# yhao-wang/DenseRetrievalToolkits

Hardware: AMD Instinct MI355X
Metric: queries/sec@top-1000, 10Mx768 corpus (BASELINE: passages encoded/sec + queries/sec@top-1000, 10Mx768 corpus, 1/2/4/8 GPU) (higher is better)
Workload: dtype bf16

## Files before the change

### denseretrievaltoolkits_amd/_native.py

```python
from __future__ import annotations

import ctypes
import os
import threading

import torch

from .build_native import LIB_PATH

DRT_OK = 0
DRT_EINVAL = -1
ROW_STATS_LEN = 34

_lock = threading.Lock()
_lib = None

c_i32 = ctypes.c_int32
c_i64 = ctypes.c_int64
c_sz = ctypes.c_size_t
c_vp = ctypes.c_void_p
c_f32 = ctypes.c_float
c_u64 = ctypes.c_uint64

_SIGNATURES = [
    ("drt_version", ctypes.c_char_p, []),
    ("drt_ip_topk_workspace", c_sz, [c_i64, c_i64, c_i32, c_i32]),
    ("drt_ip_topk_bf16", c_i32, [c_vp, c_i64, c_vp, c_i64, c_i32, c_i32, c_i64, c_vp, c_vp, c_vp, c_vp, c_sz, c_vp]),
    ("drt_ip_topk_resolve_workspace", c_sz, [c_i64, c_i64, c_i32]),
    ("drt_ip_topk_resolve", c_i32, [c_vp, c_i64, c_vp, c_i64, c_i32, c_i32, c_i64, c_vp, c_vp, c_vp, c_vp, c_sz,
                                    c_vp, c_vp]),
    ("drt_topk_merge", c_i32, [c_vp, c_vp, c_i64, c_i32, c_i32, c_i32, c_vp, c_vp, c_vp]),
    ("drt_ip_topk_sample_rank", c_i32, [c_i32]),
    ("drt_ip_topk_dist_workspace", c_sz, [c_i64, c_i64, c_i64, c_i32, c_i32]),
    ("drt_ip_topk_dist_sample", c_i32, [c_vp, c_i64, c_vp, c_i64, c_i64, c_i32, c_i32, c_vp, c_vp, c_sz, c_vp]),
    ("drt_ip_topk_dist_tau", c_i32, [c_vp, c_i64, c_i32, c_i32, c_vp, c_vp]),
    ("drt_ip_topk_dist_filter", c_i32, [c_vp, c_i64, c_vp, c_i64, c_i64, c_i32, c_i32, c_i64, c_vp, c_vp, c_vp,
                                        c_sz, c_vp]),
    ("drt_ip_topk_dist_filter_chunks", c_i32, [c_vp, c_i64, c_vp, c_i64, c_i64, c_i32, c_i32, c_i64, c_vp, c_vp,
                                               c_vp, c_i32, c_vp, c_sz, c_vp]),
    ("drt_ip_topk_tighten_rank", c_i32, [c_i64, c_i32, c_i32]),
    ("drt_ip_topk_filter_passes_workspace", c_sz, [c_i64, c_i64, c_i64, c_i32, c_i32]),
    ("drt_ip_topk_filter_passes", c_i32, [c_vp, c_i64, c_vp, c_i64, c_i64, c_i32, c_i32, c_i64, c_vp, c_vp,
                                          c_i32, c_i32, c_vp, c_vp, c_vp, c_sz, c_vp]),
    ("drt_ip_topk_dist_filter_lists", c_i32, [c_vp, c_i64, c_vp, c_i64, c_i64, c_i32, c_i32, c_i64, c_vp, c_i32,
                                              c_vp, c_vp, c_vp, c_sz, c_vp]),
    ("drt_ip_topk_dist_filter_lists_at", c_i32, [c_vp, c_i64, c_vp, c_i64, c_i64, c_i32, c_i32, c_i64, c_vp,
                                                 c_i32, c_i64, c_vp, c_vp, c_vp, c_sz, c_vp]),
    ("drt_topk_merge_packed", c_i32, [c_vp, c_i64, c_i32, c_i32, c_i64, c_vp, c_vp, c_vp, c_vp]),
    ("drt_topk_merge_packed_cert", c_i32, [c_vp, c_i64, c_i32, c_i32, c_i32, c_i64, c_vp, c_vp, c_vp, c_vp]),
    ("drt_topk_merge_packed_capped", c_i32, [c_vp, c_i64, c_i32, c_i32, c_i32, c_i32, c_i64, c_vp, c_vp, c_vp,
                                             c_vp]),
    ("drt_row_stats_bf16", c_i32, [c_vp, c_i64, c_i32, c_vp, c_i32, c_vp]),
    ("drt_refine_width", c_i32, [c_i32]),
    ("drt_ip_topk_exact_bf16", c_i32, [c_vp, c_i64, c_vp, c_i64, c_i32, c_i32, c_i64, c_vp, c_vp, c_vp, c_vp, c_vp,
                                       c_sz, c_vp]),
    ("drt_hit_metrics_i8", c_i32, [c_vp, c_i64, c_i64, c_vp, c_i32, c_vp, c_vp]),
    ("drt_answer_match_i32", c_i32, [c_vp, c_i32, c_vp, c_vp, c_i64, c_i64, c_i64, c_vp, c_vp, c_i32, c_i32, c_vp,
# ... 98 lines not shown
PROF_SCAN, PROF_SAMPLE, PROF_SELECT, PROF_MERGE, PROF_GEMM = range(5)

EXPORTED = [n for n, _, _ in _SIGNATURES]


def lib_path() -> str:
    return os.environ.get("DRT_LIB", LIB_PATH)


def load():
    global _lib
    if _lib is not None:
        return _lib
    with _lock:
        if _lib is not None:
            return _lib
        path = lib_path()
        if not os.path.exists(path):
            raise RuntimeError(
                f"DRT native library not found at {path}; build it with "
                "`python -m denseretrievaltoolkits_amd.build_native` (no CPU fallback exists)")
        lib = ctypes.CDLL(path, mode=ctypes.RTLD_LOCAL)
        for name, res, args in _SIGNATURES:
            fn = getattr(lib, name)
            fn.restype = res
            fn.argtypes = args
        _lib = lib
    return _lib


def check(rc: int, what: str) -> None:
    if rc != DRT_OK:
        if rc == DRT_EINVAL:
            raise ValueError(f"{what}: invalid argument (DRT_EINVAL)")
        raise RuntimeError(f"{what}: HIP error {rc}")


def stream_ptr(device=None) -> int:
    return torch.cuda.current_stream(device).cuda_stream
```

### denseretrievaltoolkits_amd/csrc/search.hip

```cpp
#include <cmath>

#include "profile.h"
#include "search_internal.h"

namespace drt {

constexpr int kHitCap = 1024;
constexpr int kTopRL = 4;

__host__ __device__ __forceinline__ int pass_tiles(int ntiles, int npass, int pass) {
  return npass <= 1 ? ntiles : (pass < ntiles ? (ntiles - 1 - pass) / npass + 1 : 0);
}

__device__ __forceinline__ void glds16(const void* gsrc, uint32_t lds_addr) {
  uint32_t keep;
  asm volatile(
      "s_mov_b32 %0, m0\n\t"
      "s_mov_b32 m0, %2\n\t"
      "s_nop 0\n\t"
      "global_load_lds_dwordx4 %1, off\n\t"
      "s_mov_b32 m0, %0"
      : "=&s"(keep)
      : "v"(gsrc), "s"(lds_addr)
      : "memory");
// ... 108 lines not shown
  using C = Scan16Cfg<D, NW>;
  const int rsub = lane >> 3, pos = lane & 7;
#pragma unroll
  for (int j = 0; j < C::GLDS_PER_WAVE; ++j) {
    int J = j * NW + wave;
    if (C::GLDS_PER_TILE % NW != 0) J %= C::GLDS_PER_TILE;
    const int g = J >> 1;
    const int row = ((J & 1) << 3) + rsub;
    int64_t li = tile * kT16 + row;
    li = li < a.nrows ? li : a.nrows - 1;
    const int c = pos ^ ((row >> 1) & 7);
    const __bf16* src = a.P + (a.row0 + li * a.rstride) * a.ldp + g * 64 + c * 8;
    if (NTL) glds16_nt(src, __builtin_amdgcn_readfirstlane(buf_lds + J * 1024));
    else glds16(src, __builtin_amdgcn_readfirstlane(buf_lds + J * 1024));
  }
}

template <int D, int NW>
struct LeanTile {
  using C = Scan16Cfg<D, NW>;
  static constexpr int G = C::GLDS_PER_WAVE;
  uint32_t voff[G];
  uint32_t loff[G];
  __device__ __forceinline__ void init(const ScanArgs& a, int wave, int lane) {
    const int rsub = lane >> 3, pos = lane & 7;
#pragma unroll
    for (int j = 0; j < G; ++j) {
      int J = j * NW + wave;
      if (C::GLDS_PER_TILE % NW != 0) J %= C::GLDS_PER_TILE;
      const int g = J >> 1;
      const int row = ((J & 1) << 3) + rsub;
      const int c = pos ^ ((row >> 1) & 7);
      voff[j] = (uint32_t)((row * a.ldp + g * 64 + c * 8) * 2);
      loff[j] = (uint32_t)__builtin_amdgcn_readfirstlane(J * 1024);
    }
  }
  template <bool NT>
  __device__ __forceinline__ void issue(const ScanArgs& a, uint32_t slot_lds, const char* base, bool partial,
                                        int64_t tile, int wave, int lane) {
    if (partial) {
      issue_tile16<D, NW, NT>(a, slot_lds, tile, wave, lane);
      return;
    }
#define DRT_LEAN3(POL)                                                                                   \
  {                                                                                                     \
    uint32_t keep;                                                                                      \
    asm volatile(                                                                                       \
        "s_mov_b32 %0, m0\n\t"                                                                          \
        "s_mov_b32 m0, %2\n\t"                                                                          \
        "s_nop 0\n\t"                                                                                   \
        "global_load_lds_dwordx4 %3, %1" POL "\n\t"                                                     \
        "s_mov_b32 m0, %4\n\t"                                                                          \
        "s_nop 0\n\t"                                                                                   \
        "global_load_lds_dwordx4 %5, %1" POL "\n\t"                                                     \
        "s_mov_b32 m0, %6\n\t"                                                                          \
        "s_nop 0\n\t"                                                                                   \
// ... 19 lines not shown
  }
    if constexpr (G == 3) {
      if constexpr (NT) DRT_LEAN3(" nt")
      else DRT_LEAN3("")
    } else {
#pragma unroll
      for (int j = 0; j < G; ++j) {
        if constexpr (NT) DRT_LEAN1(" nt", j)
        else DRT_LEAN1("", j)
      }
    }
#undef DRT_LEAN3
#undef DRT_LEAN1
  }
};

template <int D>
struct HalfTile {
  using C = Scan16Cfg<D, 4>;
  static constexpr bool kOk = C::GLDS_PER_TILE % 4 == 0 && C::GLDS_PER_TILE <= 24;
  static constexpr int G = C::GLDS_PER_TILE / 4;
  uint32_t voff;
  uint32_t loff;
  __device__ __forceinline__ void init(const ScanArgs& a, int wave, int lane) {
    const int lw = wave & 3;
    const int row = ((lw & 1) << 3) + (lane >> 3);
    const int c = (lane & 7) ^ ((row >> 1) & 7);
    voff = (uint32_t)((row * a.ldp + (lw >> 1) * 64 + c * 8) * 2);
    loff = (uint32_t)__builtin_amdgcn_readfirstlane(lw * 1024);
  }
  __device__ __forceinline__ void issue(const ScanArgs& a, uint32_t slot_lds, const char* base, bool partial,
                                        int tile, int wave, int lane) {
    static_assert(kOk, "loader half: a multiple of four pieces per tile");
    uint32_t v = voff;
    if (partial) {
      const int row = ((wave & 1) << 3) + (lane >> 3);
      const int last = (int)(a.nrows - 1 - (int64_t)tile * kT16);
      if (row > last) v -= (uint32_t)((row - last) * a.ldp * 2);
    }
    const uint32_t l0 = slot_lds + loff;
    uint32_t keep;
#define DRT_HALF_PIECE(LDS, OFF) \
  "s_add_u32 m0, %2, " #LDS "\n\ts_nop 0\n\tglobal_load_lds_dwordx4 %3, %1 offset:" #OFF "\n\t"
#define DRT_HALF_ISSUE(PIECES) \
  asm volatile("s_mov_b32 %0, m0\n\t" PIECES "s_mov_b32 m0, %0" : "=&s"(keep) : "s"(base), "s"(l0), "v"(v) : "memory", "scc")
#define DRT_HP0 DRT_HALF_PIECE(0, 0)
#define DRT_HP1 DRT_HP0 DRT_HALF_PIECE(3840, 256)
#define DRT_HP2 DRT_HP1 DRT_HALF_PIECE(7680, 512)
#define DRT_HP3 DRT_HP2 DRT_HALF_PIECE(11520, 768)
#define DRT_HP4 DRT_HP3 DRT_HALF_PIECE(15360, 1024)
#define DRT_HP5 DRT_HP4 DRT_HALF_PIECE(19200, 1280)
    if constexpr (G == 1) DRT_HALF_ISSUE(DRT_HP0);
    else if constexpr (G == 2) DRT_HALF_ISSUE(DRT_HP1);
    else if constexpr (G == 3) DRT_HALF_ISSUE(DRT_HP2);
    else if constexpr (G == 4) DRT_HALF_ISSUE(DRT_HP3);
    else if constexpr (G == 5) DRT_HALF_ISSUE(DRT_HP4);
    else DRT_HALF_ISSUE(DRT_HP5);
#undef DRT_HP5
#undef DRT_HP4
#undef DRT_HP3
#undef DRT_HP2
// ... 420 lines not shown
  }
  if (my_tiles & 1) epilogue(accA, rbA);
  else epilogue(accB, rbB);
  if (wcnt) wave_flush_hits(a, qw, hk, hq, wcnt, lane);
}

template <int D>
struct Scan32Cfg {
  static constexpr int KS = D / 32;
  static constexpr int RD = KS % 2 == 0 ? 2 : 1;
  static constexpr int TILE_BYTES = kT16 * D * 2;
  static constexpr int HIT_BYTES = kHitCap * 9;
  static constexpr int NB_RAW = (160 * 1024 - HIT_BYTES) / TILE_BYTES;
  static constexpr int NB = NB_RAW > 6 ? 6 : NB_RAW;
  static constexpr int RING_BYTES = NB * TILE_BYTES;
  static constexpr int LDS_BYTES = RING_BYTES + HIT_BYTES;
  static_assert(NB >= 3, "ring too small");
  static_assert(LDS_BYTES <= 160 * 1024, "LDS budget");
};
constexpr int kQueriesPerWG32 = 256;

template <int D>
__global__ __launch_bounds__(512, 1) void ip_scan32r_kernel(ScanArgs a) {
  constexpr int NW = 8;
  using C = Scan16Cfg<D, NW>;
  using C32 = Scan32Cfg<D>;
  constexpr int NB = C32::NB;
  constexpr int PD = NB - 2;
  static_assert(NB == 6, "the pair protocol's slot census");
  constexpr int KS = C32::KS;
  constexpr int RD = C32::RD;
  constexpr int kSeg = kHitCap / NW;
  __shared__ __attribute__((aligned(16))) char smem[C32::LDS_BYTES];

  const int tid = threadIdx.x;
  const int wave = __builtin_amdgcn_readfirstlane(tid >> 6);
  const int lane = tid & 63;
  const int r = lane & 15;
  const int kq = lane >> 4;
  uint64_t* hk = (uint64_t*)(smem + C32::RING_BYTES) + wave * kSeg;
  uint8_t* hq = (uint8_t*)(smem + C32::RING_BYTES + kHitCap * 8) + wave * kSeg;

  const int64_t qbase = (int64_t)blockIdx.y * kQueriesPerWG32;
  const int tmul = a.npass > 1 ? a.npass : 1;
  const int tph = a.npass > 1 ? a.pass : 0;
  const int tall = (int)((a.nrows + kT16 - 1) / kT16);
  const int ntiles = pass_tiles(tall, a.npass, a.pass);
  const uint32_t nrows = (uint32_t)a.nrows;
  const int t0 = blockIdx.x;
  const int tstep = gridDim.x;
  const int my_tiles = t0 < ntiles ? (ntiles - 1 - t0) / tstep + 1 : 0;
  if (my_tiles == 0) return;
  const int partial_tile = ((a.nrows & (kT16 - 1)) != 0 && (tall - 1) % tmul == tph) ? ntiles - 1 : -1;
  const uint32_t ring = lds_addr_of(smem);
  constexpr bool HALVES = HalfTile<D>::kOk;
  constexpr int GW = HALVES ? HalfTile<D>::G : C::GLDS_PER_WAVE;
  constexpr int KDMA = HALVES ? KS / 12 : KS / 4;
  const bool loader = !HALVES || wave >= NW / 2;
  const int64_t tile_stride = (int64_t)tstep * tmul * kT16 * a.ldp * 2;
  const char* next_base = (const char*)(a.P + ((int64_t)t0 * tmul + tph) * kT16 * a.ldp);

  const int64_t qw = qbase + wave * 32;
  bf16x8 qf0[KS], qf1[KS];
  float tau0, tau1;
  {
    const int64_t g0 = qw + r, g1 = qw + 16 + r;
    const bool ok0 = g0 < a.nq, ok1 = g1 < a.nq;
    const int64_t s0 = ok0 ? g0 : 0, s1 = ok1 ? g1 : 0;
#pragma unroll
    for (int s = 0; s < KS; ++s) {
      qf0[s] = *(const bf16x8*)(a.Q + s0 * a.ldq + s * 32 + kq * 8);
      qf1[s] = *(const bf16x8*)(a.Q + s1 * a.ldq + s * 32 + kq * 8);
    }
    const float v0 = a.tau[s0], v1 = a.tau[s1];
    tau0 = ok0 ? v0 : __builtin_nanf("");
    tau1 = ok1 ? v1 : __builtin_nanf("");
    if (!ok0) {
#pragma unroll
      for (int s = 0; s < KS; ++s) qf0[s] = (bf16x8){};
    }
    if (!ok1) {
#pragma unroll
      for (int s = 0; s < KS; ++s) qf1[s] = (bf16x8){};
    }
  }
#pragma unroll
  for (int s = 0; s < KS; ++s) asm volatile("" ::"v"(qf0[s]), "v"(qf1[s]));
  asm volatile("" ::"v"(tau0), "v"(tau1));
  asm volatile("s_waitcnt vmcnt(0)" ::: "memory");

  LeanTile<D, NW> lt;
  HalfTile<D> ht;
  if constexpr (HALVES) ht.init(a, wave, lane);
  else lt.init(a, wave, lane);
  auto issue = [&](int slot, int tile) {
    if constexpr (HALVES)
      ht.issue(a, ring + slot * C::TILE_BYTES, next_base, tile == partial_tile, tile * tmul + tph, wave, lane);
    else
      lt.template issue<false>(a, ring + slot * C::TILE_BYTES, next_base, tile == partial_tile, tile * tmul + tph,
                               wave, lane);
    next_base += tile_stride;
  };
  auto pair_wait = [&](int it) {
    if (loader && it + PD <= my_tiles) wait_vmcnt<GW>();
    else wait_vmcnt<0>();
  };
#pragma unroll
  for (int p = 0; p < PD; ++p) {
    if (p < my_tiles && loader) issue(p, t0 + p * tstep);
  }
  if (wave >= NW / 2) __builtin_amdgcn_s_setprio(1);
  pair_wait(0);
  lds_barrier();

  const int sw = (r >> 1) & 7;
  int aoff[2];
#pragma unroll
  for (int m = 0; m < 2; ++m) aoff[m] = r * 128 + (((4 * m + kq) ^ sw) << 4);
  auto frag = [&](int slot, int s) -> bf16x8 {
    return *(const bf16x8*)(smem + slot * C::TILE_BYTES + (s >> 1) * (kT16 * 128) + aoff[s & 1]);
  };
  bf16x8 af[RD];
#pragma unroll
  for (int s = 0; s < RD; ++s) af[s] = frag(0, s);

  int wcnt = 0;
  auto append = [&](const f32x4& acc, float tau, int ql, uint32_t rowbase) {
    const float mx = fmaxf(fmaxf(acc[0], acc[1]), fmaxf(acc[2], acc[3])) - tau;
    if (__ballot(mx >= 0.0f) == 0ull) return;
#pragma unroll
    for (int j = 0; j < 4; ++j) {
      const bool hit = acc[j] >= tau && rowbase + j < nrows;
      const uint64_t m = __ballot(hit);
      if (m == 0ull) continue;
      const int c = __builtin_popcountll(m);
      if (wcnt + c > kSeg) {
        wave_flush_hits(a, qw, hk, hq, wcnt, lane);
        wcnt = 0;
      }
      if (hit) {
        const int pos = wcnt + (int)__builtin_amdgcn_mbcnt_hi((uint32_t)(m >> 32),
                                                              __builtin_amdgcn_mbcnt_lo((uint32_t)m, 0u));
        hk[pos] = ((uint64_t)desc_key(acc[j]) << 32) | (uint64_t)(a.row_base + rowbase + j);
        hq[pos] = (uint8_t)ql;
      }
      wcnt += c;
    }
  };

  auto epilogue = [&](const f32x4& p0, const f32x4& p1, uint32_t rowbase) {
    append(p0, tau0, r, rowbase);
    append(p1, tau1, 16 + r, rowbase);
  };

  int buf = 0;
  auto pair_sync = [&](int it) {
    pair_wait(it);
    lds_barrier();
  };
  auto iter = [&](int it, f32x4& acc0, f32x4& acc1, uint32_t& rb, const f32x4& prev0, const f32x4& prev1,
                  uint32_t rb_prev) {
    const int tile = t0 + it * tstep;
    const bool do_dma = it + PD < my_tiles && loader;
    const int ntile = tile + PD * tstep;
    const int pslot = buf < 2 ? buf + NB - 2 : buf - 2;
    const int nslot = buf + 1 == NB ? 0 : buf + 1;
    acc0 = (f32x4){0.f, 0.f, 0.f, 0.f};
    acc1 = (f32x4){0.f, 0.f, 0.f, 0.f};
#pragma unroll
    for (int s = 0; s < KS; ++s) {
      acc0 = __builtin_amdgcn_mfma_f32_16x16x32_bf16(af[s % RD], qf0[s], acc0, 0, 0, 0);
      acc1 = __builtin_amdgcn_mfma_f32_16x16x32_bf16(af[s % RD], qf1[s], acc1, 0, 0, 0);
      af[s % RD] = s + RD < KS ? frag(buf, s + RD) : frag(nslot, s + RD - KS);
      __builtin_amdgcn_sched_barrier(0);
      if (s == KDMA && do_dma) issue(pslot, ntile);
      __builtin_amdgcn_sched_barrier(0);
    }
    if (it > 0) epilogue(prev0, prev1, rb_prev);
    rb = (uint32_t)(tile * tmul + tph) * kT16 + 4 * kq;
    buf = nslot;
  };
  f32x4 a0, a1, b0, b1;
  uint32_t rbA = 0, rbB = 0;
  for (int it = 0; it < my_tiles; it += 2) {
    if (it > 0) pair_sync(it);
    iter(it, a0, a1, rbA, b0, b1, rbB);
    if (it + 1 < my_tiles) iter(it + 1, b0, b1, rbB, a0, a1, rbA);
  }
  if (my_tiles & 1) epilogue(a0, a1, rbA);
  else epilogue(b0, b1, rbB);
  if (wcnt) wave_flush_hits(a, qw, hk, hq, wcnt, lane);
}

struct TopkPlan : PlanHead {
  int64_t n, k, nq, nq_pad;
  bool sample;
  int64_t cap;
  int64_t m;
  int64_t stride;
  int64_t r;
  int64_t nchunk;
  int64_t kc;
  size_t off_cs, off_ci, off_delta, off_rcnt, total;
};

static size_t plan_refine_tail(TopkPlan& p) {
  p.kc = refine_width(p.k);
  WsBump b{p.head_end};
  p.off_cs = b.take((size_t)p.nq_pad * p.kc * 4);
  p.off_ci = b.take((size_t)p.nq_pad * p.kc * 8);
  p.off_delta = b.take((size_t)p.nq_pad * p.kc * 4);
  p.off_rcnt = b.take((size_t)p.nq_pad * 8);
  return b.o;
}
// ... 86 lines not shown
static int scan_grid_x(int64_t ntiles) {
  int dev = 0, cus = 256;
  if (hipGetDevice(&dev) == hipSuccess) {
    int v = 0;
    if (hipDeviceGetAttribute(&v, hipDeviceAttributeMultiprocessorCount, dev) == hipSuccess && v > 0)
      cus = v;
  }
  const int64_t g = std::min<int64_t>(ntiles, (int64_t)cus);
  return (int)std::max<int64_t>(g, 1);
}

static dim3 scan16_grid(int64_t nq, int64_t nrows, int qpw = kQueriesPerWG) {
  const unsigned gy = (unsigned)((nq + qpw - 1) / qpw);
  const int64_t ntiles = (nrows + kT16 - 1) / kT16;
  int gx = scan_grid_x(ntiles);
  if (gy > 1 && ntiles >= 8) {
    const int cus = scan_grid_x((int64_t)1 << 40);
    const int share = std::max(8, (cus / (int)gy) & ~7);
    gx = (int)std::min<int64_t>(ntiles, share);
  }
  return dim3(gx, gy);
}

template <int D>
static int launch_scan_d(const ScanArgs& a, int mode, hipStream_t s) {
  if (a.nq == 0 || a.nrows == 0) return DRT_OK;
  constexpr bool kLean = D <= 768;
  if (a.npass > 1 && (mode != SCAN_FILTER || !kLean || a.row0 != 0 || a.rstride != 1 || a.pass < 0 ||
                      a.pass >= a.npass))
    return DRT_EINVAL;
  const int64_t ntiles = pass_tiles((int)((a.nrows + kT16 - 1) / kT16), a.npass, a.pass);
  if (ntiles == 0) return DRT_OK;
  const dim3 grid = scan16_grid(a.nq, ntiles * kT16);
  const unsigned gy = grid.y;
  if (mode == SCAN_FILTER) {
    const double eh = a.exp_hits > 0 ? (double)a.exp_hits : (double)a.cap / 4.0;
    const bool dense_hits = eh * 256.0 / (double)a.nrows >= 0.35;
    bool lean = false;
    if constexpr (kLean) {
      lean = a.row0 == 0 && a.rstride == 1;
      if (lean) {
        if (gy > 1) {
          const dim3 grid32 = scan16_grid(a.nq, ntiles * kT16, kQueriesPerWG32);
          hipLaunchKernelGGL((ip_scan32r_kernel<D>), grid32, dim3(512), 0, s, a);
        } else {
          hipLaunchKernelGGL((ip_scan16r_kernel<D, true>), grid, dim3(512), 0, s, a);
        }
      }
    }
    if (!lean) {
      if (dense_hits) hipLaunchKernelGGL((ip_scan16_kernel<D, SCAN_FILTER, 8, true>), grid, dim3(512), 0, s, a);
      else hipLaunchKernelGGL((ip_scan16_kernel<D, SCAN_FILTER, 8, false>), grid, dim3(512), 0, s, a);
    }
  } else if (mode == SCAN_TOPR) {
    hipLaunchKernelGGL((ip_scan16_kernel<D, SCAN_TOPR>), grid, dim3(512), 0, s, a);
  } else {
    hipLaunchKernelGGL((ip_scan16_kernel<D, SCAN_DENSE>), grid, dim3(512), 0, s, a);
  }
  return hip_status(hipGetLastError());
}

static int launch_scan_impl(const ScanArgs& a, int d, int mode, hipStream_t s) {
  switch (d) {
    case 64: return launch_scan_d<64>(a, mode, s);
    case 128: return launch_scan_d<128>(a, mode, s);
    case 192: return launch_scan_d<192>(a, mode, s);
    case 256: return launch_scan_d<256>(a, mode, s);
    case 320: return launch_scan_d<320>(a, mode, s);
    case 384: return launch_scan_d<384>(a, mode, s);
    case 448: return launch_scan_d<448>(a, mode, s);
    case 512: return launch_scan_d<512>(a, mode, s);
    case 576: return launch_scan_d<576>(a, mode, s);
    case 640: return launch_scan_d<640>(a, mode, s);
    case 704: return launch_scan_d<704>(a, mode, s);
    case 768: return launch_scan_d<768>(a, mode, s);
    case 832: return launch_scan_d<832>(a, mode, s);
    case 896: return launch_scan_d<896>(a, mode, s);
    case 960: return launch_scan_d<960>(a, mode, s);
// ... 255 lines not shown
  return resolve_impl(Q, nq, P, n, d, k, id_offset, out_scores, out_ids, status, ws, ws_bytes, n_resolved, nullptr,
                      (hipStream_t)stream);
}

int drt_ip_topk_resolve_exact(const void* Q, int64_t nq, const void* P, int64_t n, int32_t d, int32_t k,
                              int64_t id_offset, const float* stats, float* out_scores, int64_t* out_ids,
                              int32_t* status, void* ws, size_t ws_bytes, int64_t* n_resolved, void* stream) {
  DRT_REQUIRE(stats != nullptr);
  return resolve_impl(Q, nq, P, n, d, k, id_offset, out_scores, out_ids, status, ws, ws_bytes, n_resolved, stats,
                      (hipStream_t)stream);
}

int32_t drt_ip_topk_sample_rank(int32_t k) {
  if (k < 1 || k > kSelMaxK) return -1;
  const TopkPlan p = make_plan(1, (int64_t)0xFFFFFFFEll, k);
  return (int32_t)p.r;
}

size_t drt_ip_topk_dist_workspace(int64_t nq, int64_t n_local, int64_t n_global, int32_t d, int32_t k) {
  if (!valid_dist_dims(nq, n_local, n_global, d, k)) return 0;
  return make_dist_plan(nq, n_local, n_global, k).total;
}

int drt_ip_topk_dist_sample(const void* Q, int64_t nq, const void* P, int64_t n_local, int64_t n_global, int32_t d,
                            int32_t k, uint32_t* best, void* ws, size_t ws_bytes, void* stream) {
  DRT_REQUIRE(valid_dist_dims(nq, n_local, n_global, d, k));
  if (nq == 0) return DRT_OK;
  DRT_REQUIRE(Q && best && ws);
  const TopkPlan p = make_dist_plan(nq, n_local, n_global, k);
  DRT_REQUIRE(ws_bytes >= p.total);
  const int64_t r = drt_ip_topk_sample_rank(k);
  hipStream_t s = (hipStream_t)stream;
  if (!p.sample || n_local == 0) {
    DRT_CHECK_HIP(hipMemsetAsync(best, 0xFF, (size_t)nq * r * 4, s));
    return DRT_OK;
  }
  DRT_REQUIRE(P != nullptr);
  char* w = (char*)ws;
  ScanArgs a = scan_args(Q, nq, P, d);
  a.row0 = p.stride / 2;
  a.nrows = p.m;
  a.rstride = p.stride;
  a.out = w + p.off_sample;
  const int64_t nlists = 4 * (int64_t)scan16_grid(nq, p.m).x;
  if (nlists * kTopRL <= kKthChunk && nlists * kTopRL <= align_up(p.m, 4)) {
    a.cap = nlists * kTopRL;
    DRT_CHECK_HIP(hipMemsetAsync(a.out, 0xFF, (size_t)nq * a.cap * 4, s));
    int rc = launch_scan(a, d, SCAN_TOPR, s, PROF_SAMPLE);
    if (rc) return rc;
    const ProfPair pp = prof_begin(PROF_SELECT, s);
    launch_kth_final(nq, (const uint32_t*)a.out, (int)nlists, (int)r, (int64_t)kTopRL, (int64_t)a.cap, nullptr, best,
                     nullptr, kTopRL, s);
    prof_end(pp, s);
    return hip_status(hipGetLastError());
  }
  a.cap = align_up(p.m, 4);
  int rc = launch_scan(a, d, SCAN_DENSE, s, PROF_SAMPLE);
  if (rc) return rc;
  const ProfPair pp = prof_begin(PROF_SELECT, s);
  launch_kth_partial(p.nchunk, nq, (const uint32_t*)(w + p.off_sample), (int64_t)align_up(p.m, 4), p.m, (int)r,
                     (uint32_t*)(w + p.off_part), s);
  launch_kth_final(nq, (const uint32_t*)(w + p.off_part), (int)p.nchunk, (int)r, (int64_t)r, (int64_t)(p.nchunk * r),
                   nullptr, best, nullptr, (int)r, s);
  prof_end(pp, s);
  return hip_status(hipGetLastError());
}

int drt_ip_topk_dist_tau(const uint32_t* lists, int64_t nq, int32_t nlists, int32_t k, float* tau, void* stream) {
// ... 192 lines not shown
```

### denseretrievaltoolkits_amd/kernels.py

```python
from __future__ import annotations

from typing import Optional, Tuple

import torch

from . import _native, ops


def _require_device(*ts: torch.Tensor) -> None:
    for t in ts:
        if not t.is_cuda:
            raise ValueError("DRT kernels run on the GPU only (got a CPU tensor; no CPU fallback exists)")


def ip_topk_workspace_bytes(nq: int, n: int, d: int, k: int) -> int:
    return int(_native.load().drt_ip_topk_workspace(nq, n, d, k))


def ip_topk(q: torch.Tensor, p: torch.Tensor, k: int, id_offset: int = 0, resolve: bool = True,
            out: Optional[Tuple[torch.Tensor, torch.Tensor]] = None,
            status: Optional[torch.Tensor] = None,
            stats: Optional[torch.Tensor] = None) -> Tuple[torch.Tensor, torch.Tensor, torch.Tensor]:
    drt = ops.load()
    _require_device(q, p)
# ... 192 lines not shown
        all_reduce_sum(delta)
    return drt.refine_sort(cand_s, cand_i, delta, cnt, k)


def topk_merge(scores: torch.Tensor, ids: torch.Tensor, k_out: int) -> Tuple[torch.Tensor, torch.Tensor]:
    _require_device(scores, ids)
    if scores.dim() != 3 or scores.shape != ids.shape:
        raise ValueError("topk_merge expects [nparts, nq, k] scores and ids")
    return ops.load().topk_merge(scores.float(), ids.long(), k_out)


def sample_rank(k: int) -> int:
    r = int(_native.load().drt_ip_topk_sample_rank(k))
    if r <= 0:
        raise ValueError(f"unsupported k={k}")
    return r


def dist_sample(q: torch.Tensor, p: torch.Tensor, n_global: int, k: int) -> torch.Tensor:
    _require_device(q, p)
    return ops.load().dist_sample(q, p, n_global, k)


def dist_tau(lists: torch.Tensor, k: int) -> torch.Tensor:
    _require_device(lists)
    return ops.load().dist_tau(lists, k)


def dist_filter(q: torch.Tensor, p: torch.Tensor, n_global: int, k: int, id_offset: int,
                tau: torch.Tensor) -> torch.Tensor:
    _require_device(q, p, tau)
    return ops.load().dist_filter(q, p, n_global, k, id_offset, tau)


def dist_filter_lists(q: torch.Tensor, p: torch.Tensor, n_global: int, k: int, id_offset: int,
                      lists: torch.Tensor) -> torch.Tensor:
    _require_device(q, p, lists)
    return ops.load().dist_filter_lists(q, p, n_global, k, id_offset, lists)


def dist_filter_into(q: torch.Tensor, p: torch.Tensor, n_global: int, k: int, id_offset: int, tau: torch.Tensor,
                     packed: torch.Tensor) -> None:
    _require_device(q, p, tau, packed)
    ops.load().dist_filter_into(q, p, n_global, k, id_offset, tau, packed)


# ... 104 lines not shown
```

### include/drt.h

```cpp
#ifndef DRT_H_
#define DRT_H_

#include <stddef.h>
#include <stdint.h>

#ifdef __cplusplus
extern "C" {
#endif

#define DRT_OK 0
#define DRT_EINVAL (-1)
#define DRT_ROW_STATS_LEN 34

const char* drt_version(void);

size_t drt_ip_topk_workspace(int64_t nq, int64_t n, int32_t d, int32_t k);
int drt_ip_topk_bf16(const void* Q, int64_t nq, const void* P, int64_t n, int32_t d,
                     int32_t k, int64_t id_offset, float* out_scores, int64_t* out_ids,
                     int32_t* status, void* workspace, size_t workspace_bytes,
                     void* stream);

size_t drt_ip_topk_resolve_workspace(int64_t n_failed, int64_t n, int32_t d);
int drt_ip_topk_resolve(const void* Q, int64_t nq, const void* P, int64_t n, int32_t d,
                        int32_t k, int64_t id_offset, float* out_scores, int64_t* out_ids,
// ... 43 lines not shown
                       void* stream);

int drt_topk_merge(const float* scores, const int64_t* ids, int64_t nq, int32_t nparts,
                   int32_t k_in, int32_t k_out, float* out_scores, int64_t* out_ids,
                   void* stream);

int drt_topk_exclude(const float* scores, const int64_t* ids, int64_t nq, int32_t k_in, const int64_t* excl,
                     const int64_t* excl_off, const float* ceiling, int32_t skip, int32_t k_out,
                     float* out_scores, int64_t* out_ids, int32_t* out_count, void* stream);
int drt_pair_scores_bf16(const void* Q, int64_t nq, const void* P, int64_t n, int32_t d, const int32_t* qidx,
                         const int64_t* rows, int64_t npairs, float* out, void* stream);

size_t drt_topk_collapse_workspace(int64_t nq, int32_t k_in);
int drt_topk_collapse(const float* scores, const int64_t* ids, int64_t nq, int32_t k_in, const int32_t* groups,
                      int64_t n_rows, int32_t k_out, float* out_scores, int32_t* out_groups, int64_t* out_ids,
                      int32_t* out_count, void* workspace, size_t workspace_bytes, void* stream);

int32_t drt_ip_topk_sample_rank(int32_t k);
size_t drt_ip_topk_dist_workspace(int64_t nq, int64_t n_local, int64_t n_global, int32_t d,
                                  int32_t k);
int drt_ip_topk_dist_sample(const void* Q, int64_t nq, const void* P, int64_t n_local,
                            int64_t n_global, int32_t d, int32_t k, uint32_t* best, void* ws,
                            size_t ws_bytes, void* stream);
int drt_ip_topk_dist_tau(const uint32_t* lists, int64_t nq, int32_t nlists, int32_t k, float* tau,
                         void* stream);
int drt_ip_topk_dist_filter(const void* Q, int64_t nq, const void* P, int64_t n_local,
                            int64_t n_global, int32_t d, int32_t k, int64_t id_offset,
                            const float* tau, uint64_t* packed, void* ws, size_t ws_bytes,
                            void* stream);
int drt_ip_topk_dist_filter_chunks(const void* Q, int64_t nq, const void* P, int64_t n_local,
                                   int64_t n_global, int32_t d, int32_t k, int64_t id_offset,
                                   const float* tau, uint64_t* packed, const int64_t* starts,
                                   int32_t nchunks, void* ws, size_t ws_bytes, void* stream);
int32_t drt_ip_topk_tighten_rank(int64_t n_local, int32_t npasses, int32_t k);
size_t drt_ip_topk_filter_passes_workspace(int64_t nq, int64_t n_local, int64_t n_global, int32_t d,
                                           int32_t k);
int drt_ip_topk_filter_passes(const void* Q, int64_t nq, const void* P, int64_t n_local,
                              int64_t n_global, int32_t d, int32_t k, int64_t id_offset,
                              const float* tau, uint64_t* packed, int32_t npasses, int32_t r,
                              float* tau1_out, uint32_t* pass0_out, void* ws, size_t ws_bytes,
                              void* stream);
int drt_ip_topk_dist_filter_lists(const void* Q, int64_t nq, const void* P, int64_t n_local,
                                  int64_t n_global, int32_t d, int32_t k, int64_t id_offset,
                                  const uint32_t* lists, int32_t nlists, float* tau_out,
                                  uint64_t* packed, void* ws, size_t ws_bytes, void* stream);
int drt_ip_topk_dist_filter_lists_at(const void* Q, int64_t nq, const void* P, int64_t n_local,
// ... 156 lines not shown
```

Baseline: 89130.

## Route top-R sampling scan through the 32-query lean pipelined kernel

Moves the scan32r kernel body into a shared header so it can be built in both filter and top-R modes. The sampling pass (SCAN_TOPR) now uses the 32-queries-per-workgroup MFMA pipeline, with strided row loads and a per-lane top-4 bubble. The aim is a faster sample/threshold stage than the older scan16 top-R kernel. The sample list count now comes from the new grid, and a query function for that count is exported; this changes how many candidate lists the tau stage sees.

```diff
diff --git a/denseretrievaltoolkits_amd/_native.py b/denseretrievaltoolkits_amd/_native.py
--- a/denseretrievaltoolkits_amd/_native.py
+++ b/denseretrievaltoolkits_amd/_native.py
@@ -33,6 +33,7 @@
     ("drt_ip_topk_sample_rank", c_i32, [c_i32]),
     ("drt_ip_topk_dist_workspace", c_sz, [c_i64, c_i64, c_i64, c_i32, c_i32]),
     ("drt_ip_topk_dist_sample", c_i32, [c_vp, c_i64, c_vp, c_i64, c_i64, c_i32, c_i32, c_vp, c_vp, c_sz, c_vp]),
+    ("drt_ip_topk_dist_sample_lists", c_i32, [c_i64, c_i64, c_i64, c_i32, c_i32]),
     ("drt_ip_topk_dist_tau", c_i32, [c_vp, c_i64, c_i32, c_i32, c_vp, c_vp]),
     ("drt_ip_topk_dist_filter", c_i32, [c_vp, c_i64, c_vp, c_i64, c_i64, c_i32, c_i32, c_i64, c_vp, c_vp, c_vp,
                                         c_sz, c_vp]),
@@ -177,6 +178,8 @@
                 "`python -m denseretrievaltoolkits_amd.build_native` (no CPU fallback exists)")
         lib = ctypes.CDLL(path, mode=ctypes.RTLD_LOCAL)
         for name, res, args in _SIGNATURES:
+            if path != LIB_PATH and not hasattr(lib, name):
+                continue
             fn = getattr(lib, name)
             fn.restype = res
             fn.argtypes = args
diff --git a/denseretrievaltoolkits_amd/csrc/scan32r_body.h b/denseretrievaltoolkits_amd/csrc/scan32r_body.h
--- /dev/null
+++ b/denseretrievaltoolkits_amd/csrc/scan32r_body.h
@@ -0,0 +1,210 @@
+  constexpr bool TOPR = MODE == SCAN_TOPR;
+  constexpr int NW = 8;
+  using C = Scan16Cfg<D, NW>;
+  using C32 = Scan32Cfg<D>;
+  constexpr int NB = C32::NB;
+  constexpr int PD = NB - 2;
+  static_assert(NB == 6, "the pair protocol's slot census");
+  constexpr int KS = C32::KS;
+  constexpr int RD = C32::RD;
+  constexpr int kSeg = kHitCap / NW;
+  __shared__ __attribute__((aligned(16))) char smem[C32::LDS_BYTES];
+
+  const int tid = threadIdx.x;
+  const int wave = __builtin_amdgcn_readfirstlane(tid >> 6);
+  const int lane = tid & 63;
+  const int r = lane & 15;
+  const int kq = lane >> 4;
+  uint64_t* hk = (uint64_t*)(smem + C32::RING_BYTES) + wave * kSeg;
+  uint8_t* hq = (uint8_t*)(smem + C32::RING_BYTES + kHitCap * 8) + wave * kSeg;
+
+  const int64_t qbase = (int64_t)blockIdx.y * kQueriesPerWG32;
+  const int tmul = a.npass > 1 ? a.npass : 1;
+  const int tph = a.npass > 1 ? a.pass : 0;
+  const int tall = (int)((a.nrows + kT16 - 1) / kT16);
+  const int ntiles = pass_tiles(tall, a.npass, a.pass);
+  const uint32_t nrows = (uint32_t)a.nrows;
+  const int t0 = blockIdx.x;
+  const int tstep = gridDim.x;
+  const int my_tiles = t0 < ntiles ? (ntiles - 1 - t0) / tstep + 1 : 0;
+  if (my_tiles == 0) return;
+  const int partial_tile = ((a.nrows & (kT16 - 1)) != 0 && (tall - 1) % tmul == tph) ? ntiles - 1 : -1;
+  const uint32_t ring = lds_addr_of(smem);
+  constexpr bool HALVES = HalfTile<D>::kOk;
+  constexpr int GW = HALVES ? HalfTile<D>::G : C::GLDS_PER_WAVE;
+  constexpr int KDMA = HALVES ? KS / 12 : KS / 4;
+  const bool loader = !HALVES || wave >= NW / 2;
+  int64_t tile_stride = (int64_t)tstep * tmul * kT16 * a.ldp * 2;
+  const char* next_base = (const char*)(a.P + ((int64_t)t0 * tmul + tph) * kT16 * a.ldp);
+  if constexpr (TOPR) {
+    tile_stride *= a.rstride;
+    next_base = (const char*)(a.P + (a.row0 + (int64_t)t0 * kT16 * a.rstride) * a.ldp);
+  }
+
+  const int64_t qw = qbase + wave * 32;
+  bf16x8 qf0[KS], qf1[KS];
+  float tau0, tau1;
+  {
+    const int64_t g0 = qw + r, g1 = qw + 16 + r;
+    const bool ok0 = g0 < a.nq, ok1 = g1 < a.nq;
+    const int64_t s0 = ok0 ? g0 : 0, s1 = ok1 ? g1 : 0;
+#pragma unroll
+    for (int s = 0; s < KS; ++s) {
+      qf0[s] = *(const bf16x8*)(a.Q + s0 * a.ldq + s * 32 + kq * 8);
+      qf1[s] = *(const bf16x8*)(a.Q + s1 * a.ldq + s * 32 + kq * 8);
+    }
+    if constexpr (TOPR) {
+      tau0 = tau1 = 0.f;
+    } else {
+      const float v0 = a.tau[s0], v1 = a.tau[s1];
+      tau0 = ok0 ? v0 : __builtin_nanf("");
+      tau1 = ok1 ? v1 : __builtin_nanf("");
+    }
+    if (!ok0) {
+#pragma unroll
+      for (int s = 0; s < KS; ++s) qf0[s] = (bf16x8){};
+    }
+    if (!ok1) {
+#pragma unroll
+      for (int s = 0; s < KS; ++s) qf1[s] = (bf16x8){};
+    }
+  }
+#pragma unroll
+  for (int s = 0; s < KS; ++s) asm volatile("" ::"v"(qf0[s]), "v"(qf1[s]));
+  asm volatile("" ::"v"(tau0), "v"(tau1));
+  asm volatile("s_waitcnt vmcnt(0)" ::: "memory");
+
+  LeanTile<D, NW> lt;
+  HalfTile<D> ht;
+  if constexpr (HALVES) ht.template init<TOPR>(a, wave, lane);
+  else lt.template init<TOPR>(a, wave, lane);
+  auto issue = [&](int slot, int tile) {
+    if constexpr (HALVES)
+      ht.template issue<TOPR>(a, ring + slot * C::TILE_BYTES, next_base, tile == partial_tile, tile * tmul + tph, wave,
+                              lane);
+    else
+      lt.template issue<false>(a, ring + slot * C::TILE_BYTES, next_base, tile == partial_tile, tile * tmul + tph,
+                               wave, lane);
+    next_base += tile_stride;
+  };
+  auto pair_wait = [&](int it) {
+    if (loader && it + PD <= my_tiles) wait_vmcnt<GW>();
+    else wait_vmcnt<0>();
+  };
+#pragma unroll
+  for (int p = 0; p < PD; ++p) {
+    if (p < my_tiles && loader) issue(p, t0 + p * tstep);
+  }
+  if (wave >= NW / 2) __builtin_amdgcn_s_setprio(1);
+  pair_wait(0);
+  lds_barrier();
+
+  const int sw = (r >> 1) & 7;
+  int aoff[2];
+#pragma unroll
+  for (int m = 0; m < 2; ++m) aoff[m] = r * 128 + (((4 * m + kq) ^ sw) << 4);
+  auto frag = [&](int slot, int s) -> bf16x8 {
+    return *(const bf16x8*)(smem + slot * C::TILE_BYTES + (s >> 1) * (kT16 * 128) + aoff[s & 1]);
+  };
+  bf16x8 af[RD];
+#pragma unroll
+  for (int s = 0; s < RD; ++s) af[s] = frag(0, s);
+
+  int wcnt = 0;
+  auto append = [&](const f32x4& acc, float tau, int ql, uint32_t rowbase) {
+    const float mx = fmaxf(fmaxf(acc[0], acc[1]), fmaxf(acc[2], acc[3])) - tau;
+    if (__ballot(mx >= 0.0f) == 0ull) return;
+#pragma unroll
+    for (int j = 0; j < 4; ++j) {
+      const bool hit = acc[j] >= tau && rowbase + j < nrows;
+      const uint64_t m = __ballot(hit);
+      if (m == 0ull) continue;
+      const int c = __builtin_popcountll(m);
+      if (wcnt + c > kSeg) {
+        wave_flush_hits(a, qw, hk, hq, wcnt, lane);
+        wcnt = 0;
+      }
+      if (hit) {
+        const int pos = wcnt + (int)__builtin_amdgcn_mbcnt_hi((uint32_t)(m >> 32),
+                                                              __builtin_amdgcn_mbcnt_lo((uint32_t)m, 0u));
+        hk[pos] = ((uint64_t)desc_key(acc[j]) << 32) | (uint64_t)(a.row_base + rowbase + j);
+        hq[pos] = (uint8_t)ql;
+      }
+      wcnt += c;
+    }
+  };
+
+  uint32_t top0[TOPR ? kTopRL : 1], top1[TOPR ? kTopRL : 1];
+#pragma unroll
+  for (int i = 0; i < (TOPR ? kTopRL : 1); ++i) top0[i] = top1[i] = 0xFFFFFFFFu;
+  auto bubble = [&](uint32_t (&top)[TOPR ? kTopRL : 1], const f32x4& acc, uint32_t rowbase) {
+#pragma unroll
+    for (int j = 0; j < 4; ++j) {
+      uint32_t x = rowbase + j < nrows ? desc_key(acc[j]) : 0xFFFFFFFFu;
+#pragma unroll
+      for (int i = 0; i < (TOPR ? kTopRL : 1); ++i) {
+        const uint32_t lo = x < top[i] ? x : top[i];
+        x = x < top[i] ? top[i] : x;
+        top[i] = lo;
+      }
+    }
+  };
+  auto epilogue = [&](const f32x4& p0, const f32x4& p1, uint32_t rowbase) {
+    if constexpr (TOPR) {
+      bubble(top0, p0, rowbase);
+      bubble(top1, p1, rowbase);
+    } else {
+      append(p0, tau0, r, rowbase);
+      append(p1, tau1, 16 + r, rowbase);
+    }
+  };
+
+  int buf = 0;
+  auto pair_sync = [&](int it) {
+    pair_wait(it);
+    lds_barrier();
+  };
+  auto iter = [&](int it, f32x4& acc0, f32x4& acc1, uint32_t& rb, const f32x4& prev0, const f32x4& prev1,
+                  uint32_t rb_prev) {
+    const int tile = t0 + it * tstep;
+    const bool do_dma = it + PD < my_tiles && loader;
+    const int ntile = tile + PD * tstep;
+    const int pslot = buf < 2 ? buf + NB - 2 : buf - 2;
+    const int nslot = buf + 1 == NB ? 0 : buf + 1;
+    acc0 = (f32x4){0.f, 0.f, 0.f, 0.f};
+    acc1 = (f32x4){0.f, 0.f, 0.f, 0.f};
+#pragma unroll
+    for (int s = 0; s < KS; ++s) {
+      acc0 = __builtin_amdgcn_mfma_f32_16x16x32_bf16(af[s % RD], qf0[s], acc0, 0, 0, 0);
+      acc1 = __builtin_amdgcn_mfma_f32_16x16x32_bf16(af[s % RD], qf1[s], acc1, 0, 0, 0);
+      af[s % RD] = s + RD < KS ? frag(buf, s + RD) : frag(nslot, s + RD - KS);
+      __builtin_amdgcn_sched_barrier(0);
+      if (s == KDMA && do_dma) issue(pslot, ntile);
+      __builtin_amdgcn_sched_barrier(0);
+    }
+    if (it > 0) epilogue(prev0, prev1, rb_prev);
+    rb = (uint32_t)(tile * tmul + tph) * kT16 + 4 * kq;
+    buf = nslot;
+  };
+  f32x4 a0, a1, b0, b1;
+  uint32_t rbA = 0, rbB = 0;
+  for (int it = 0; it < my_tiles; it += 2) {
+    if (it > 0) pair_sync(it);
+    iter(it, a0, a1, rbA, b0, b1, rbB);
+    if (it + 1 < my_tiles) iter(it + 1, b0, b1, rbB, a0, a1, rbA);
+  }
+  if (my_tiles & 1) epilogue(a0, a1, rbA);
+  else epilogue(b0, b1, rbB);
+  if constexpr (TOPR) {
+    uint32_t* o = (uint32_t*)a.out + ((int64_t)blockIdx.x * 4 + kq) * kTopRL;
+    if (qw + r < a.nq) {
+#pragma unroll
+      for (int i = 0; i < kTopRL; ++i) o[(qw + r) * a.cap + i] = top0[i];
+    }
+    if (qw + 16 + r < a.nq) {
+#pragma unroll
+      for (int i = 0; i < kTopRL; ++i) o[(qw + 16 + r) * a.cap + i] = top1[i];
+    }
+  } else {
+    if (wcnt) wave_flush_hits(a, qw, hk, hq, wcnt, lane);
+  }
diff --git a/denseretrievaltoolkits_amd/csrc/search.hip b/denseretrievaltoolkits_amd/csrc/search.hip
--- a/denseretrievaltoolkits_amd/csrc/search.hip
+++ b/denseretrievaltoolkits_amd/csrc/search.hip
@@ -154,8 +154,10 @@
   static constexpr int G = C::GLDS_PER_WAVE;
   uint32_t voff[G];
   uint32_t loff[G];
+  template <bool STR = false>
   __device__ __forceinline__ void init(const ScanArgs& a, int wave, int lane) {
     const int rsub = lane >> 3, pos = lane & 7;
+    const int64_t pitch = STR ? a.ldp * a.rstride : a.ldp;
 #pragma unroll
     for (int j = 0; j < G; ++j) {
       int J = j * NW + wave;
@@ -163,7 +165,7 @@
       const int g = J >> 1;
       const int row = ((J & 1) << 3) + rsub;
       const int c = pos ^ ((row >> 1) & 7);
-      voff[j] = (uint32_t)((row * a.ldp + g * 64 + c * 8) * 2);
+      voff[j] = (uint32_t)((row * pitch + g * 64 + c * 8) * 2);
       loff[j] = (uint32_t)__builtin_amdgcn_readfirstlane(J * 1024);
     }
   }
@@ -229,13 +231,16 @@
   static constexpr int G = C::GLDS_PER_TILE / 4;
   uint32_t voff;
   uint32_t loff;
+  template <bool STR = false>
   __device__ __forceinline__ void init(const ScanArgs& a, int wave, int lane) {
     const int lw = wave & 3;
     const int row = ((lw & 1) << 3) + (lane >> 3);
     const int c = (lane & 7) ^ ((row >> 1) & 7);
-    voff = (uint32_t)((row * a.ldp + (lw >> 1) * 64 + c * 8) * 2);
+    const int64_t pitch = STR ? a.ldp * a.rstride : a.ldp;
+    voff = (uint32_t)((row * pitch + (lw >> 1) * 64 + c * 8) * 2);
     loff = (uint32_t)__builtin_amdgcn_readfirstlane(lw * 1024);
   }
+  template <bool STR = false>
   __device__ __forceinline__ void issue(const ScanArgs& a, uint32_t slot_lds, const char* base, bool partial,
                                         int tile, int wave, int lane) {
     static_assert(kOk, "loader half: a multiple of four pieces per tile");
@@ -243,7 +248,8 @@
     if (partial) {
       const int row = ((wave & 1) << 3) + (lane >> 3);
       const int last = (int)(a.nrows - 1 - (int64_t)tile * kT16);
-      if (row > last) v -= (uint32_t)((row - last) * a.ldp * 2);
+      const int64_t pitch = STR ? a.ldp * a.rstride : a.ldp;
+      if (row > last) v -= (uint32_t)((row - last) * pitch * 2);
     }
     const uint32_t l0 = slot_lds + loff;
     uint32_t keep;
@@ -710,174 +716,14 @@
 
 template <int D>
 __global__ __launch_bounds__(512, 1) void ip_scan32r_kernel(ScanArgs a) {
-  constexpr int NW = 8;
-  using C = Scan16Cfg<D, NW>;
-  using C32 = Scan32Cfg<D>;
-  constexpr int NB = C32::NB;
-  constexpr int PD = NB - 2;
-  static_assert(NB == 6, "the pair protocol's slot census");
-  constexpr int KS = C32::KS;
-  constexpr int RD = C32::RD;
-  constexpr int kSeg = kHitCap / NW;
-  __shared__ __attribute__((aligned(16))) char smem[C32::LDS_BYTES];
-
-  const int tid = threadIdx.x;
-  const int wave = __builtin_amdgcn_readfirstlane(tid >> 6);
-  const int lane = tid & 63;
-  const int r = lane & 15;
-  const int kq = lane >> 4;
-  uint64_t* hk = (uint64_t*)(smem + C32::RING_BYTES) + wave * kSeg;
-  uint8_t* hq = (uint8_t*)(smem + C32::RING_BYTES + kHitCap * 8) + wave * kSeg;
-
-  const int64_t qbase = (int64_t)blockIdx.y * kQueriesPerWG32;
-  const int tmul = a.npass > 1 ? a.npass : 1;
-  const int tph = a.npass > 1 ? a.pass : 0;
-  const int tall = (int)((a.nrows + kT16 - 1) / kT16);
-  const int ntiles = pass_tiles(tall, a.npass, a.pass);
-  const uint32_t nrows = (uint32_t)a.nrows;
-  const int t0 = blockIdx.x;
-  const int tstep = gridDim.x;
-  const int my_tiles = t0 < ntiles ? (ntiles - 1 - t0) / tstep + 1 : 0;
-  if (my_tiles == 0) return;
-  const int partial_tile = ((a.nrows & (kT16 - 1)) != 0 && (tall - 1) % tmul == tph) ? ntiles - 1 : -1;
-  const uint32_t ring = lds_addr_of(smem);
-  constexpr bool HALVES = HalfTile<D>::kOk;
-  constexpr int GW = HALVES ? HalfTile<D>::G : C::GLDS_PER_WAVE;
-  constexpr int KDMA = HALVES ? KS / 12 : KS / 4;
-  const bool loader = !HALVES || wave >= NW / 2;
-  const int64_t tile_stride = (int64_t)tstep * tmul * kT16 * a.ldp * 2;
-  const char* next_base = (const char*)(a.P + ((int64_t)t0 * tmul + tph) * kT16 * a.ldp);
-
-  const int64_t qw = qbase + wave * 32;
-  bf16x8 qf0[KS], qf1[KS];
-  float tau0, tau1;
-  {
-    const int64_t g0 = qw + r, g1 = qw + 16 + r;
-    const bool ok0 = g0 < a.nq, ok1 = g1 < a.nq;
-    const int64_t s0 = ok0 ? g0 : 0, s1 = ok1 ? g1 : 0;
-#pragma unroll
-    for (int s = 0; s < KS; ++s) {
-      qf0[s] = *(const bf16x8*)(a.Q + s0 * a.ldq + s * 32 + kq * 8);
-      qf1[s] = *(const bf16x8*)(a.Q + s1 * a.ldq + s * 32 + kq * 8);
-    }
-    const float v0 = a.tau[s0], v1 = a.tau[s1];
-    tau0 = ok0 ? v0 : __builtin_nanf("");
-    tau1 = ok1 ? v1 : __builtin_nanf("");
-    if (!ok0) {
-#pragma unroll
-      for (int s = 0; s < KS; ++s) qf0[s] = (bf16x8){};
-    }
-    if (!ok1) {
-#pragma unroll
-      for (int s = 0; s < KS; ++s) qf1[s] = (bf16x8){};
-    }
-  }
-#pragma unroll
-  for (int s = 0; s < KS; ++s) asm volatile("" ::"v"(qf0[s]), "v"(qf1[s]));
-  asm volatile("" ::"v"(tau0), "v"(tau1));
-  asm volatile("s_waitcnt vmcnt(0)" ::: "memory");
-
-  LeanTile<D, NW> lt;
-  HalfTile<D> ht;
-  if constexpr (HALVES) ht.init(a, wave, lane);
-  else lt.init(a, wave, lane);
-  auto issue = [&](int slot, int tile) {
-    if constexpr (HALVES)
-      ht.issue(a, ring + slot * C::TILE_BYTES, next_base, tile == partial_tile, tile * tmul + tph, wave, lane);
-    else
-      lt.template issue<false>(a, ring + slot * C::TILE_BYTES, next_base, tile == partial_tile, tile * tmul + tph,
-                               wave, lane);
-    next_base += tile_stride;
-  };
-  auto pair_wait = [&](int it) {
-    if (loader && it + PD <= my_tiles) wait_vmcnt<GW>();
-    else wait_vmcnt<0>();
-  };
-#pragma unroll
-  for (int p = 0; p < PD; ++p) {
-    if (p < my_tiles && loader) issue(p, t0 + p * tstep);
-  }
-  if (wave >= NW / 2) __builtin_amdgcn_s_setprio(1);
-  pair_wait(0);
-  lds_barrier();
-
-  const int sw = (r >> 1) & 7;
-  int aoff[2];
-#pragma unroll
-  for (int m = 0; m < 2; ++m) aoff[m] = r * 128 + (((4 * m + kq) ^ sw) << 4);
-  auto frag = [&](int slot, int s) -> bf16x8 {
-    return *(const bf16x8*)(smem + slot * C::TILE_BYTES + (s >> 1) * (kT16 * 128) + aoff[s & 1]);
-  };
-  bf16x8 af[RD];
-#pragma unroll
-  for (int s = 0; s < RD; ++s) af[s] = frag(0, s);
-
-  int wcnt = 0;
-  auto append = [&](const f32x4& acc, float tau, int ql, uint32_t rowbase) {
-    const float mx = fmaxf(fmaxf(acc[0], acc[1]), fmaxf(acc[2], acc[3])) - tau;
-    if (__ballot(mx >= 0.0f) == 0ull) return;
-#pragma unroll
-    for (int j = 0; j < 4; ++j) {
-      const bool hit = acc[j] >= tau && rowbase + j < nrows;
-      const uint64_t m = __ballot(hit);
-      if (m == 0ull) continue;
-      const int c = __builtin_popcountll(m);
-      if (wcnt + c > kSeg) {
-        wave_flush_hits(a, qw, hk, hq, wcnt, lane);
-        wcnt = 0;
-      }
-      if (hit) {
-        const int pos = wcnt + (int)__builtin_amdgcn_mbcnt_hi((uint32_t)(m >> 32),
-                                                              __builtin_amdgcn_mbcnt_lo((uint32_t)m, 0u));
-        hk[pos] = ((uint64_t)desc_key(acc[j]) << 32) | (uint64_t)(a.row_base + rowbase + j);
-        hq[pos] = (uint8_t)ql;
-      }
-      wcnt += c;
-    }
-  };
-
-  auto epilogue = [&](const f32x4& p0, const f32x4& p1, uint32_t rowbase) {
-    append(p0, tau0, r, rowbase);
-    append(p1, tau1, 16 + r, rowbase);
-  };
-
-  int buf = 0;
-  auto pair_sync = [&](int it) {
-    pair_wait(it);
-    lds_barrier();
-  };
-  auto iter = [&](int it, f32x4& acc0, f32x4& acc1, uint32_t& rb, const f32x4& prev0, const f32x4& prev1,
-                  uint32_t rb_prev) {
-    const int tile = t0 + it * tstep;
-    const bool do_dma = it + PD < my_tiles && loader;
-    const int ntile = tile + PD * tstep;
-    const int pslot = buf < 2 ? buf + NB - 2 : buf - 2;
-    const int nslot = buf + 1 == NB ? 0 : buf + 1;
-    acc0 = (f32x4){0.f, 0.f, 0.f, 0.f};
-    acc1 = (f32x4){0.f, 0.f, 0.f, 0.f};
-#pragma unroll
-    for (int s = 0; s < KS; ++s) {
-      acc0 = __builtin_amdgcn_mfma_f32_16x16x32_bf16(af[s % RD], qf0[s], acc0, 0, 0, 0);
-      acc1 = __builtin_amdgcn_mfma_f32_16x16x32_bf16(af[s % RD], qf1[s], acc1, 0, 0, 0);
-      af[s % RD] = s + RD < KS ? frag(buf, s + RD) : frag(nslot, s + RD - KS);
-      __builtin_amdgcn_sched_barrier(0);
-      if (s == KDMA && do_dma) issue(pslot, ntile);
-      __builtin_amdgcn_sched_barrier(0);
-    }
-    if (it > 0) epilogue(prev0, prev1, rb_prev);
-    rb = (uint32_t)(tile * tmul + tph) * kT16 + 4 * kq;
-    buf = nslot;
-  };
-  f32x4 a0, a1, b0, b1;
-  uint32_t rbA = 0, rbB = 0;
-  for (int it = 0; it < my_tiles; it += 2) {
-    if (it > 0) pair_sync(it);
-    iter(it, a0, a1, rbA, b0, b1, rbB);
-    if (it + 1 < my_tiles) iter(it + 1, b0, b1, rbB, a0, a1, rbA);
-  }
-  if (my_tiles & 1) epilogue(a0, a1, rbA);
-  else epilogue(b0, b1, rbB);
-  if (wcnt) wave_flush_hits(a, qw, hk, hq, wcnt, lane);
+  constexpr int MODE = SCAN_FILTER;
+#include "scan32r_body.h"
+}
+
+template <int D>
+__global__ __launch_bounds__(512, 1) void ip_scan32r_topr_kernel(ScanArgs a) {
+  constexpr int MODE = SCAN_TOPR;
+#include "scan32r_body.h"
 }
 
 struct TopkPlan : PlanHead {
@@ -1010,6 +856,13 @@
   return dim3(gx, gy);
 }
 
+static bool topr_lean32(int64_t nq, int d, int64_t ldp, int64_t rstride) {
+  return nq > kQueriesPerWG && d <= 768 && ldp * rstride <= ((int64_t)1 << 26);
+}
+static dim3 topr_grid(int64_t nq, int64_t nrows, int d, int64_t ldp, int64_t rstride) {
+  return scan16_grid(nq, nrows, topr_lean32(nq, d, ldp, rstride) ? kQueriesPerWG32 : kQueriesPerWG);
+}
+
 template <int D>
 static int launch_scan_d(const ScanArgs& a, int mode, hipStream_t s) {
   if (a.nq == 0 || a.nrows == 0) return DRT_OK;
@@ -1041,7 +894,14 @@
       else hipLaunchKernelGGL((ip_scan16_kernel<D, SCAN_FILTER, 8, false>), grid, dim3(512), 0, s, a);
     }
   } else if (mode == SCAN_TOPR) {
-    hipLaunchKernelGGL((ip_scan16_kernel<D, SCAN_TOPR>), grid, dim3(512), 0, s, a);
+    bool lean32 = false;
+    if constexpr (kLean) {
+      lean32 = topr_lean32(a.nq, D, a.ldp, a.rstride);
+      if (lean32)
+        hipLaunchKernelGGL((ip_scan32r_topr_kernel<D>), topr_grid(a.nq, a.nrows, D, a.ldp, a.rstride), dim3(512), 0, s,
+                           a);
+    }
+    if (!lean32) hipLaunchKernelGGL((ip_scan16_kernel<D, SCAN_TOPR>), grid, dim3(512), 0, s, a);
   } else {
     hipLaunchKernelGGL((ip_scan16_kernel<D, SCAN_DENSE>), grid, dim3(512), 0, s, a);
   }
@@ -1343,6 +1203,17 @@
   return make_dist_plan(nq, n_local, n_global, k).total;
 }
 
+static int64_t topr_sample_lists(const TopkPlan& p, int64_t nq, int32_t d) {
+  if (!p.sample || p.m == 0 || nq == 0) return 0;
+  const int64_t nlists = 4 * (int64_t)topr_grid(nq, p.m, d, d, p.stride).x;
+  return nlists * kTopRL <= kKthChunk && nlists * kTopRL <= (int64_t)align_up(p.m, 4) ? nlists : 0;
+}
+
+int32_t drt_ip_topk_dist_sample_lists(int64_t nq, int64_t n_local, int64_t n_global, int32_t d, int32_t k) {
+  if (!valid_dist_dims(nq, n_local, n_global, d, k)) return -1;
+  return (int32_t)topr_sample_lists(make_dist_plan(nq, n_local, n_global, k), nq, d);
+}
+
 int drt_ip_topk_dist_sample(const void* Q, int64_t nq, const void* P, int64_t n_local, int64_t n_global, int32_t d,
                             int32_t k, uint32_t* best, void* ws, size_t ws_bytes, void* stream) {
   DRT_REQUIRE(valid_dist_dims(nq, n_local, n_global, d, k));
@@ -1363,8 +1234,8 @@
   a.nrows = p.m;
   a.rstride = p.stride;
   a.out = w + p.off_sample;
-  const int64_t nlists = 4 * (int64_t)scan16_grid(nq, p.m).x;
-  if (nlists * kTopRL <= kKthChunk && nlists * kTopRL <= align_up(p.m, 4)) {
+  const int64_t nlists = topr_sample_lists(p, nq, d);
+  if (nlists > 0) {
     a.cap = nlists * kTopRL;
     DRT_CHECK_HIP(hipMemsetAsync(a.out, 0xFF, (size_t)nq * a.cap * 4, s));
     int rc = launch_scan(a, d, SCAN_TOPR, s, PROF_SAMPLE);
diff --git a/denseretrievaltoolkits_amd/kernels.py b/denseretrievaltoolkits_amd/kernels.py
--- a/denseretrievaltoolkits_amd/kernels.py
+++ b/denseretrievaltoolkits_amd/kernels.py
@@ -238,6 +238,13 @@
     return ops.load().dist_sample(q, p, n_global, k)
 
 
+def dist_sample_lists(nq: int, n_local: int, n_global: int, d: int, k: int) -> int:
+    n = int(_native.load().drt_ip_topk_dist_sample_lists(nq, n_local, n_global, d, k))
+    if n < 0:
+        raise ValueError("dist_sample_lists: invalid dimensions")
+    return n
+
+
 def dist_tau(lists: torch.Tensor, k: int) -> torch.Tensor:
     _require_device(lists)
     return ops.load().dist_tau(lists, k)
diff --git a/include/drt.h b/include/drt.h
--- a/include/drt.h
+++ b/include/drt.h
@@ -89,6 +89,7 @@
 int drt_ip_topk_dist_sample(const void* Q, int64_t nq, const void* P, int64_t n_local,
                             int64_t n_global, int32_t d, int32_t k, uint32_t* best, void* ws,
                             size_t ws_bytes, void* stream);
+int32_t drt_ip_topk_dist_sample_lists(int64_t nq, int64_t n_local, int64_t n_global, int32_t d, int32_t k);
 int drt_ip_topk_dist_tau(const uint32_t* lists, int64_t nq, int32_t nlists, int32_t k, float* tau,
                          void* stream);
 int drt_ip_topk_dist_filter(const void* Q, int64_t nq, const void* P, int64_t n_local,
```

After: 89540, median of 6. About the same (+0.5%).
